# bingjeff/trex-gym

Measured on NVIDIA B200. Metric: env-steps/sec at 65,536 envs/GPU, higher is better.
Workload: dtype f32

## Files before the change

### trex_gym_b200/csrc/trex_core.h

```cpp
#pragma once
#include "trex_topology.h"
#include <stddef.h>

#ifndef TREX_KMAX
#define TREX_KMAX 16
#endif
#ifndef TREX_PGS_UNROLL
#define TREX_PGS_UNROLL TREX_ROLLED
#endif
#define TREX_NCAND_MAX 64
#define TREX_MAX_ROUNDS 12
#ifdef TREX_PHASES
#define TREX_STATE_STRIDE 176
#else
#define TREX_STATE_STRIDE 160
#endif
#define W_COL 0
#define W_RHSM 992
#define W_JDI 1024
#define W_DSELF 1056
#define W_RHSL 1088
#define W_SIGMA 1120
#define TREX_KC 8
#define W_NC 1152
#define W_CS 1160
#define W_BT (W_CS + 16 * TREX_KC)
#define W_A4 (W_BT + 96 * TREX_KC)
#define TREX_WORK_STRIDE 2848
static_assert(W_A4 + 12 * TREX_KC * TREX_KC <= TREX_WORK_STRIDE && (W_BT % 4) == 0 && (W_A4 % 4) == 0 && (TREX_WORK_STRIDE % 32) == 0,
              "work record layout");
#define TREX_KW TREX_KMAX
#define H_NC 0
#define H_CS 8
#define H_BT (H_CS + 16 * TREX_KW)
#define H_A4 (H_BT + 96 * TREX_KW)
#define TREX_HEAVY_STRIDE (((H_A4 + 9 * TREX_KW * TREX_KW) + 31) / 32 * 32)
static_assert((H_BT % 4) == 0 && (H_A4 % 4) == 0 && TREX_KC <= TREX_KW, "heavy record layout");
#define TREX_NCLASS 6
#define TREX_CLASS_HEAVY (TREX_NCLASS - 1)
TREX_TOPO_FN int defer_class(int n_contacts) {
  return n_contacts <= 2 ? n_contacts : (n_contacts <= 4 ? 3 : (n_contacts <= TREX_KC ? 4 : TREX_CLASS_HEAVY));
}
#ifdef TREX_PHASES
#define TREX_AUX_STRIDE 16
#define TREX_TICK(i) { const long long _t = cycle_count(); stats.phase[i] += (float)(_t - _t0); _t0 = _t; }
#else
#define TREX_AUX_STRIDE 8
#define TREX_TICK(i)
#endif

namespace trex {

using trex_topo::NB;
using trex_topo::NJ;
using trex_topo::MAX_DEPTH;

enum {
  F_E0 = 0,
  F_R0 = 9,
  F_MASS = 12,
  F_MC = 13,
  F_I = 16,
  F_DROT = 22,
  F_LOWER = 28,
  F_UPPER = 29,
  F_JDAMP = 30,
  F_STARTQ = 31,
  F_COUNT = 32
};
enum {
  IF_PARENT_LANE = 0,
  IF_DEPTH = 1,
  IF_ANC_MASK = 2,
  IF_CHILDREN = 3,
  IF_OBS_SLOT = 4,
  IF_DAMP_LANE = 5,
  IF_DAMP_CONTRIB = 6,
  IF_LIMIT_ORDER = 7,
  IF_LEVEL = 8,
  IF_COUNT = 8 + MAX_DEPTH
};

struct Uniform {
  float dt, g, kp, kd, max_impulse, k_lin, k_ang, maxvel, erp, contact_erp, split_thresh, slop;
  float resid_thresh, warm, mu, breaking, floor_z, limit_max_impulse, reset_z, target_h;
  float w_dist, w_energy, w_drift;
  float head_p[3];
  float r0[NB][3];
  int iters, n_sub, max_episode_steps, head_lane, n_cand, n_rounds, contacts_on, reset_mode;
  int defer_contacts;
  unsigned seed;
  long long env_offset;
  float reset_z_min, reset_z_max;
  unsigned char order[2 * NJ];
  unsigned char depth[NB];
  unsigned char max_children[MAX_DEPTH + 1];
  unsigned char head_chain[MAX_DEPTH];
  int head_depth;
};

struct alignas(16) WarpShared {
  float col[31][32];
  float tmp[1][32];
  float lam_cache[TREX_NCAND_MAX];
  float cpos[TREX_KMAX][4];
  int ccand[TREX_KMAX];
  int clane[TREX_KMAX];
  union {
    struct {
      float E[9][32];
      float U[6][32];
      float invD[32];
      float Rw[9][32];
      float xw[3][32];
      float pack[32][16];
    } k;
    struct {
      float dV[3 * TREX_KMAX][32];
      float Jc[3 * TREX_KMAX][12];
      unsigned char slot[TREX_KMAX][32];
      unsigned char inv[TREX_KW][16];
    } c;
    struct {
      float keep[28][32];
      float pA[6][32];
      float cc[5][32];
      float uu[32];
      float Ip[21][32];
      float pp[6][32];
      float base[32];
    } x;
  };
};
static_assert(sizeof(((WarpShared*)0)->x) <= sizeof(((WarpShared*)0)->c), "exchange area must fit the union");
static_assert(sizeof(((WarpShared*)0)->x.keep) == 28 * 128, "exchange area must start behind k.E .. k.xw");
#define TREX_PART_ROW 44
static_assert(sizeof(((WarpShared*)0)->k) <= TREX_PART_ROW * 128, "partials must not overlap the kinematics arrays");
static_assert(sizeof(((WarpShared*)0)->c) >= (TREX_PART_ROW + 6) * 128, "contact-row storage too small for the damping scratch");

TREX_FN constexpr int SI(int i, int j) {
  return (i <= j) ? (i * 6 - (i * (i - 1)) / 2 + (j - i)) : (j * 6 - (j * (j - 1)) / 2 + (i - j));
}
TREX_FN constexpr int body_lane(int b) { return b == 0 ? 25 : b - 1; }

struct EnvRegs {
  vf q, qd, tgt, tau;
  float pos[3], quat[4], om[3], vl[3];
};

TREX_FN uint32_t sig_mix_u(uint32_t h, uint32_t w) { return (h ^ w) * 16777619u; }
#define TREX_CONE_EDGE 0.9999f

struct StepStats {
  uint32_t sig;
  int iters;
  int contacts;
  int overflow;
#ifdef TREX_PHASES
  float phase[8];
#endif
};

#define MDL(f) ldg_ro(mdl, lane + (f) * 32)
#define MDLI(f) ldi(mdli, lane + (f) * 32)

TREX_FN vf clampv(vf x, float lo, float hi) { return sel(x < lo, lo, sel(x > hi, hi, x)); }
TREX_FN float clampf(float x, float lo, float hi) { return x < lo ? lo : (x > hi ? hi : x); }

TREX_FN void quat_to_Rb(const float q[4], float Rb[9]) {
  const float x = q[0], y = q[1], z = q[2], w = q[3];
  const float s = 2.0f / (x * x + y * y + z * z + w * w);
  Rb[0] = 1.0f - s * (y * y + z * z); Rb[3] = s * (x * y - w * z);        Rb[6] = s * (x * z + w * y);
  Rb[1] = s * (x * y + w * z);        Rb[4] = 1.0f - s * (x * x + z * z); Rb[7] = s * (y * z - w * x);
  Rb[2] = s * (x * z - w * y);        Rb[5] = s * (y * z + w * x);        Rb[8] = 1.0f - s * (x * x + y * y);
}

TREX_FN void local_rotation(const float* mdl, vi lane, vf q, vf E[9]) {
  const vf c = vcos(q), s = vsin(q);
  vf e0[9];
  TREX_UNROLL for (int k = 0; k < 9; k++) e0[k] = MDL(F_E0 + k);
  E[0] = c * e0[0] + s * e0[1]; E[1] = c * e0[3] + s * e0[4]; E[2] = c * e0[6] + s * e0[7];
  E[3] = c * e0[1] - s * e0[0]; E[4] = c * e0[4] - s * e0[3]; E[5] = c * e0[7] - s * e0[6];
  E[6] = e0[2]; E[7] = e0[5]; E[8] = e0[8];
}

template <bool WITH_VEL>
TREX_FN void forward_pass(const float* mdl, const int* mdli, vi lane, const EnvRegs& R, const float Rb[9],
                          const vf E[9], vf Rw[9], vf xw[3], vf v[6]) {
  const vi plane = MDLI(IF_PARENT_LANE);
  const vi depth = MDLI(IF_DEPTH);
  vf r0[3];
  TREX_UNROLL for (int k = 0; k < 3; k++) r0[k] = MDL(F_R0 + k);
  TREX_UNROLL for (int k = 0; k < 9; k++) Rw[k] = vbroadcast(Rb[k]);
  TREX_UNROLL for (int k = 0; k < 3; k++) xw[k] = vbroadcast(R.pos[k]);
  if (WITH_VEL) {
    TREX_UNROLL for (int i = 0; i < 3; i++) {
      v[i] = vbroadcast(Rb[3 * i] * R.om[0] + Rb[3 * i + 1] * R.om[1] + Rb[3 * i + 2] * R.om[2]);
      v[3 + i] = vbroadcast(Rb[3 * i] * R.vl[0] + Rb[3 * i + 1] * R.vl[1] + Rb[3 * i + 2] * R.vl[2]);
    }
  }
  TREX_ROLLED for (int d = 1; d <= MAX_DEPTH; d++) {
    const vb at = depth == d;
    vf pR[9], px[3];
    TREX_UNROLL for (int k = 0; k < 9; k++) pR[k] = shflv(Rw[k], plane);
    TREX_UNROLL for (int k = 0; k < 3; k++) px[k] = shflv(xw[k], plane);
    TREX_UNROLL for (int i = 0; i < 3; i++)
      TREX_UNROLL for (int j = 0; j < 3; j++) {
        const vf t = E[3 * i] * pR[j] + E[3 * i + 1] * pR[3 + j] + E[3 * i + 2] * pR[6 + j];
        Rw[3 * i + j] = sel(at, t, Rw[3 * i + j]);
      }
    TREX_UNROLL for (int j = 0; j < 3; j++) {
      const vf t = px[j] + pR[j] * r0[0] + pR[3 + j] * r0[1] + pR[6 + j] * r0[2];
      xw[j] = sel(at, t, xw[j]);
    }
    if (WITH_VEL) {
      vf pv[6];
      TREX_UNROLL for (int k = 0; k < 6; k++) pv[k] = shflv(v[k], plane);
      const vf lx = pv[3] + (pv[1] * r0[2] - pv[2] * r0[1]);
      const vf ly = pv[4] + (pv[2] * r0[0] - pv[0] * r0[2]);
      const vf lz = pv[5] + (pv[0] * r0[1] - pv[1] * r0[0]);
      TREX_UNROLL for (int i = 0; i < 3; i++) {
        vf wa = E[3 * i] * pv[0] + E[3 * i + 1] * pv[1] + E[3 * i + 2] * pv[2];
        const vf la = E[3 * i] * lx + E[3 * i + 1] * ly + E[3 * i + 2] * lz;
        if (i == 2) wa = wa + R.qd;
        v[i] = sel(at, wa, v[i]);
        v[3 + i] = sel(at, la, v[3 + i]);
      }
    }
  }
}

struct Chol6 {
  float L[6][6];
  float rd[6];
};
TREX_FN void spd6_factor(const float a[21], Chol6& c) {
  TREX_UNROLL for (int j = 0; j < 6; j++) {
    float s = a[SI(j, j)];
    TREX_UNROLL for (int k = 0; k < j; k++) s -= c.L[j][k] * c.L[j][k];
    const float id = 1.0f / sqrtf(s);
    c.rd[j] = id;
    TREX_UNROLL for (int i = j + 1; i < 6; i++) {
      float t = a[SI(i, j)];
      TREX_UNROLL for (int k = 0; k < j; k++) t -= c.L[i][k] * c.L[j][k];
      c.L[i][j] = t * id;
    }
  }
}
template <class T>
TREX_FN void spd6_solve_neg(const Chol6& c, const T b[6], T x[6]) {
  T y[6];
  TREX_UNROLL for (int i = 0; i < 6; i++) {
    T t = b[i];
    TREX_UNROLL for (int k = 0; k < i; k++) t = t - y[k] * c.L[i][k];
    y[i] = t * c.rd[i];
  }
  TREX_UNROLL for (int i = 5; i >= 0; i--) {
    T t = y[i];
    TREX_UNROLL for (int k = i + 1; k < 6; k++) t = t - x[k] * c.L[k][i];
    x[i] = t * c.rd[i];
  }
  TREX_UNROLL for (int i = 0; i < 6; i++) x[i] = -x[i];
}

TREX_FN void to_parent(const vf E[9], const vf r[3], const vf Ia[21], const vf pa[6], vf Ip[21], vf pp[6]) {
  vf Ar[3][3], Br[3][3], Mr[3][3];
  {
    const vf a00 = Ia[SI(0, 0)], a01 = Ia[SI(0, 1)], a11 = Ia[SI(1, 1)];
    vf T0[3], T1[3];
    TREX_UNROLL for (int j = 0; j < 3; j++) {
      T0[j] = a00 * E[j] + a01 * E[3 + j];
      T1[j] = a01 * E[j] + a11 * E[3 + j];
    }
    TREX_UNROLL for (int i = 0; i < 3; i++)
      TREX_UNROLL for (int j = i; j < 3; j++) Ar[i][j] = E[i] * T0[j] + E[3 + i] * T1[j];
  }
  {
    vf T0[3], T1[3];
    TREX_UNROLL for (int j = 0; j < 3; j++) {
      T0[j] = Ia[SI(0, 3)] * E[j] + Ia[SI(0, 4)] * E[3 + j] + Ia[SI(0, 5)] * E[6 + j];
      T1[j] = Ia[SI(1, 3)] * E[j] + Ia[SI(1, 4)] * E[3 + j] + Ia[SI(1, 5)] * E[6 + j];
    }
    TREX_UNROLL for (int i = 0; i < 3; i++)
      TREX_UNROLL for (int j = 0; j < 3; j++) Br[i][j] = E[i] * T0[j] + E[3 + i] * T1[j];
  }
  {
    vf T[3][3];
    TREX_UNROLL for (int i = 0; i < 3; i++)
      TREX_UNROLL for (int j = 0; j < 3; j++)
        T[i][j] = Ia[SI(3 + i, 3)] * E[j] + Ia[SI(3 + i, 4)] * E[3 + j] + Ia[SI(3 + i, 5)] * E[6 + j];
    TREX_UNROLL for (int i = 0; i < 3; i++)
      TREX_UNROLL for (int j = i; j < 3; j++) {
        Mr[i][j] = E[i] * T[0][j] + E[3 + i] * T[1][j] + E[6 + i] * T[2][j];
        Mr[j][i] = Mr[i][j];
      }
  }
  vf K[3][3], C[3][3], Dm[3][3], Bp[3][3];
  TREX_UNROLL for (int j = 0; j < 3; j++) {
    K[0][j] = r[1] * Mr[2][j] - r[2] * Mr[1][j];
    K[1][j] = r[2] * Mr[0][j] - r[0] * Mr[2][j];
    K[2][j] = r[0] * Mr[1][j] - r[1] * Mr[0][j];
  }
  TREX_UNROLL for (int i = 0; i < 3; i++)
    TREX_UNROLL for (int j = 0; j < 3; j++) Bp[i][j] = Br[i][j] + K[i][j];
  TREX_UNROLL for (int j = 0; j < 3; j++) {
    C[0][j] = r[1] * Br[j][2] - r[2] * Br[j][1];
    C[1][j] = r[2] * Br[j][0] - r[0] * Br[j][2];
    C[2][j] = r[0] * Br[j][1] - r[1] * Br[j][0];
    Dm[0][j] = r[1] * Bp[j][2] - r[2] * Bp[j][1];
    Dm[1][j] = r[2] * Bp[j][0] - r[0] * Bp[j][2];
    Dm[2][j] = r[0] * Bp[j][1] - r[1] * Bp[j][0];
  }
  TREX_UNROLL for (int i = 0; i < 3; i++)
    TREX_UNROLL for (int j = i; j < 3; j++) {
      Ip[SI(i, j)] = Ar[i][j] + C[i][j] + Dm[j][i];
      Ip[SI(3 + i, 3 + j)] = Mr[i][j];
    }
  TREX_UNROLL for (int i = 0; i < 3; i++)
    TREX_UNROLL for (int j = 0; j < 3; j++) Ip[SI(i, 3 + j)] = Bp[i][j];
  vf fn[3], ff[3];
  TREX_UNROLL for (int i = 0; i < 3; i++) {
    fn[i] = E[i] * pa[0] + E[3 + i] * pa[1] + E[6 + i] * pa[2];
    ff[i] = E[i] * pa[3] + E[3 + i] * pa[4] + E[6 + i] * pa[5];
  }
  pp[0] = fn[0] + (r[1] * ff[2] - r[2] * ff[1]);
  pp[1] = fn[1] + (r[2] * ff[0] - r[0] * ff[2]);
  pp[2] = fn[2] + (r[0] * ff[1] - r[1] * ff[0]);
  pp[3] = ff[0]; pp[4] = ff[1]; pp[5] = ff[2];
}

TREX_FN void finish_substep(const Uniform& P, vi lane, EnvRegs& R, vf dv, vf lam_m) {
  const vb is_joint = lane < NJ;
  const float dt = P.dt;
  R.qd = sel(is_joint, clampv(R.qd + dv, -P.maxvel, P.maxvel), 0.0f);
  TREX_UNROLL for (int k = 0; k < 3; k++) {
    R.om[k] = clampf(R.om[k] + lane_value(dv, 25 + k), -P.maxvel, P.maxvel);
    R.vl[k] = clampf(R.vl[k] + lane_value(dv, 28 + k), -P.maxvel, P.maxvel);
  }
  R.tau = sel(is_joint, vdiv(lam_m, dt), 0.0f);
  TREX_UNROLL for (int k = 0; k < 3; k++) R.pos[k] += dt * R.vl[k];
  {
    float fAngle = sqrtf(R.om[0] * R.om[0] + R.om[1] * R.om[1] + R.om[2] * R.om[2]);
    if (fAngle * dt > 0.78539816339744831f) fAngle = 0.78539816339744831f / dt;
    float sc;
    if (fAngle < 0.001f) sc = 0.5f * dt - (dt * dt * dt) * 0.020833333333f * fAngle * fAngle;
    else sc = sinf(0.5f * fAngle * dt) / fAngle;
    const float ax = R.om[0] * sc, ay = R.om[1] * sc, az = R.om[2] * sc, aw = cosf(fAngle * dt * 0.5f);
    const float x = R.quat[0], y = R.quat[1], z = R.quat[2], w = R.quat[3];
    const float nx = aw * x + ax * w + ay * z - az * y;
    const float ny = aw * y - ax * z + ay * w + az * x;
    const float nz = aw * z + ax * y - ay * x + az * w;
    const float nw = aw * w - ax * x - ay * y - az * z;
    const float inv = 1.0f / sqrtf(nx * nx + ny * ny + nz * nz + nw * nw);
    R.quat[0] = nx * inv; R.quat[1] = ny * inv; R.quat[2] = nz * inv; R.quat[3] = nw * inv;
  }
  R.q = sel(is_joint, R.q + dt * R.qd, 0.0f);
}

TREX_FN void inward_packed(const Uniform& P, const float* mdl, const int* mdli, WarpShared* slabs, int valid_mask) {
  const vi lane = lane_id();
  const vi e = lane >> 3, i = lane & 7;
  const vb env_ok = ((vi(valid_mask) >> e) & 1) != 0;
  float* sb = reinterpret_cast<float*>(slabs);
  const vi eo = e * (int)(sizeof(WarpShared) / sizeof(float));
  constexpr int O_E = offsetof(WarpShared, k.E) / 4, O_U = offsetof(WarpShared, k.U) / 4, O_ID = offsetof(WarpShared, k.invD) / 4;
  constexpr int O_PA = offsetof(WarpShared, x.pA) / 4, O_CC = offsetof(WarpShared, x.cc) / 4, O_UU = offsetof(WarpShared, x.uu) / 4;
  constexpr int O_IP = offsetof(WarpShared, x.Ip) / 4, O_PP = offsetof(WarpShared, x.pp) / 4, O_BASE = offsetof(WarpShared, x.base) / 4;
  vi blv[MAX_DEPTH + 1];
  blv[0] = seli(i == 0, vi(25), vi(-1));
  TREX_UNROLL for (int d = 1; d <= MAX_DEPTH; d++) blv[d] = ldi(mdli, i + (IF_LEVEL + d - 1) * 32);
  vf n_mass, n_mc[3], n_I3[6], n_r0[3];
  vi n_children;
#define TREX_LOAD_LEVEL_CONSTANTS(BL)                                                       \
  {                                                                                         \
    const vi b_ = (BL);                                                                     \
    n_mass = ldg_ro(mdl, b_ + F_MASS * 32);                                                 \
    TREX_UNROLL for (int k = 0; k < 3; k++) n_mc[k] = ldg_ro(mdl, b_ + (F_MC + k) * 32);    \
    TREX_UNROLL for (int k = 0; k < 6; k++) n_I3[k] = ldg_ro(mdl, b_ + (F_I + k) * 32);     \
    TREX_UNROLL for (int k = 0; k < 3; k++) n_r0[k] = ldg_ro(mdl, b_ + (F_R0 + k) * 32);    \
    n_children = ldi(mdli, b_ + IF_CHILDREN * 32);                                          \
  }
  TREX_LOAD_LEVEL_CONSTANTS(seli(env_ok && (blv[MAX_DEPTH] >= 0), blv[MAX_DEPTH], 0))
  TREX_ROLLED for (int d = MAX_DEPTH; d >= 0; d--) {
    vi bl0 = blv[0], bln = blv[0];
    TREX_UNROLL for (int dd = 1; dd <= MAX_DEPTH; dd++) {
      bl0 = seli(vi(d) == dd, blv[dd], bl0);
      bln = seli(vi(d) == dd + 1, blv[dd], bln);
    }
    const vb has = env_ok && (bl0 >= 0);
    const vi bl = seli(has, bl0, 0);
    vf mc[3], I3[6], r0[3], pA[6];
    const vf mass = n_mass;
    const vi children = n_children;
    TREX_UNROLL for (int k = 0; k < 3; k++) { mc[k] = n_mc[k]; r0[k] = n_r0[k]; }
    TREX_UNROLL for (int k = 0; k < 6; k++) I3[k] = n_I3[k];
    if (d > 0) TREX_LOAD_LEVEL_CONSTANTS(seli(env_ok && (bln >= 0), bln, 0))
    TREX_UNROLL for (int k = 0; k < 6; k++) pA[k] = ld(sb, eo + bl + (O_PA + k * 32));
    vf IA[21];
    TREX_UNROLL for (int k = 0; k < 21; k++) IA[k] = 0.0f;
    IA[SI(0, 0)] = I3[0]; IA[SI(0, 1)] = I3[1]; IA[SI(0, 2)] = I3[2];
    IA[SI(1, 1)] = I3[3]; IA[SI(1, 2)] = I3[4]; IA[SI(2, 2)] = I3[5];
    IA[SI(0, 4)] = -mc[2]; IA[SI(0, 5)] = mc[1];
    IA[SI(1, 3)] = mc[2];  IA[SI(1, 5)] = -mc[0];
    IA[SI(2, 3)] = -mc[1]; IA[SI(2, 4)] = mc[0];
    IA[SI(3, 3)] = mass; IA[SI(4, 4)] = mass; IA[SI(5, 5)] = mass;
    if (d < MAX_DEPTH) {
      const int nslots = P.max_children[d];
      TREX_ROLLED for (int sidx = 0; sidx < nslots; sidx++) {
        const vi cl = (children >> (6 * sidx)) & 63;
        const vb ok = has && (cl != 63);
        const vi cls = seli(ok, cl, bl);
        TREX_UNROLL for (int k = 0; k < 21; k++) IA[k] = IA[k] + sel(ok, ld(sb, eo + cls + (O_IP + k * 32)), 0.0f);
        TREX_UNROLL for (int k = 0; k < 6; k++) pA[k] = pA[k] + sel(ok, ld(sb, eo + cls + (O_PP + k * 32)), 0.0f);
      }
    }
    if (d == 0) {
      TREX_UNROLL for (int k = 0; k < 21; k++) st_if(sb, eo + (O_BASE + k), IA[k], has);
      TREX_UNROLL for (int k = 0; k < 6; k++) st_if(sb, eo + (O_BASE + 21 + k), pA[k], has);
      break;
    }
    vf E[9];
    TREX_UNROLL for (int k = 0; k < 9; k++) E[k] = ld(sb, eo + bl + (O_E + k * 32));
    const vf c0 = ld(sb, eo + bl + O_CC), c1 = ld(sb, eo + bl + (O_CC + 32)), c3 = ld(sb, eo + bl + (O_CC + 64)),
             c4 = ld(sb, eo + bl + (O_CC + 96)), tau_j = ld(sb, eo + bl + (O_CC + 128));
    vf Ut[6];
    Ut[0] = IA[SI(0, 2)]; Ut[1] = IA[SI(1, 2)]; Ut[2] = IA[SI(2, 2)];
    Ut[3] = IA[SI(2, 3)]; Ut[4] = IA[SI(2, 4)]; Ut[5] = IA[SI(2, 5)];
    const vf Dt = Ut[2];
    const vb okD = Dt >= 1.1920929e-7f;
    const vf iD = sel(okD, vdiv(1.0f, sel(okD, Dt, 1.0f)), 0.0f);
    const vf ut = tau_j - pA[2];
    TREX_UNROLL for (int k = 0; k < 6; k++) st_if(sb, eo + bl + (O_U + k * 32), Ut[k], has);
    st_if(sb, eo + bl + O_ID, iD, has);
    st_if(sb, eo + bl + O_UU, ut, has);
    vf Ia[21];
    TREX_UNROLL for (int a = 0; a < 6; a++)
      TREX_UNROLL for (int b = a; b < 6; b++) Ia[SI(a, b)] = IA[SI(a, b)] - (Ut[a] * iD) * Ut[b];
    vf pa[6];
    const vf s = ut * iD;
    TREX_UNROLL for (int a = 0; a < 6; a++)
      pa[a] = a == 2 ? pA[a] + Ut[a] * s : pA[a] + (Ia[SI(a, 0)] * c0 + Ia[SI(a, 1)] * c1 + Ia[SI(a, 3)] * c3 + Ia[SI(a, 4)] * c4) + Ut[a] * s;
    vf Ip[21], pp[6];
    to_parent(E, r0, Ia, pa, Ip, pp);
    TREX_UNROLL for (int k = 0; k < 21; k++) st_if(sb, eo + bl + (O_IP + k * 32), Ip[k], has);
    TREX_UNROLL for (int k = 0; k < 6; k++) st_if(sb, eo + bl + (O_PP + k * 32), pp[k], has);
    warp_sync();
  }
#undef TREX_LOAD_LEVEL_CONSTANTS
  warp_sync();
}

template <bool PACKED = false>
TREX_FN int substep(const Uniform& P, const float* mdl, const int* mdli, const float* tasks, const float* cand_p,
                     const int* cand_lane, WarpShared& S, EnvRegs& R, float kp, float kd, float max_imp,
                     StepStats& stats, float* work, WarpShared* cta_slabs = nullptr, int warp_in_cta = 0, int valid_mask = 0,
                     float* workh = nullptr) {
  const vi lane = lane_id();
  const vb is_joint = lane < NJ;
  const vb is_base = lane == 25;
  const vi plane = MDLI(IF_PARENT_LANE);
  const vi depth = MDLI(IF_DEPTH);
  const vi anc = MDLI(IF_ANC_MASK);
  const float dt = P.dt;

#ifdef TREX_PHASES
  long long _t0 = cycle_count();
#endif
  float Rb[9];
  quat_to_Rb(R.quat, Rb);

  vf E[9];
  local_rotation(mdl, lane, R.q, E);
  TREX_UNROLL for (int k = 0; k < 9; k++) E[k] = sel(is_base, vbroadcast(Rb[k]), E[k]);
  vf Rw[9], xw[3], v[6];
  forward_pass<true>(mdl, mdli, lane, R, Rb, E, Rw, xw, v);
  TREX_UNROLL for (int k = 0; k < 9; k++) { st(S.k.E[k], lane, E[k]); st(S.k.Rw[k], lane, Rw[k]); }
  TREX_UNROLL for (int k = 0; k < 3; k++) st(S.k.xw[k], lane, xw[k]);

  TREX_TICK(0)
  const vf mass = MDL(F_MASS);
  vf mc[3], I3[6];
  TREX_UNROLL for (int k = 0; k < 3; k++) mc[k] = MDL(F_MC + k);
  TREX_UNROLL for (int k = 0; k < 6; k++) I3[k] = MDL(F_I + k);
  vf pA[6];
  {
    const vf wx = v[0], wy = v[1], wz = v[2], lx = v[3], ly = v[4], lz = v[5];
    const vf nx = I3[0] * wx + I3[1] * wy + I3[2] * wz + (mc[1] * lz - mc[2] * ly);
    const vf ny = I3[1] * wx + I3[3] * wy + I3[4] * wz + (mc[2] * lx - mc[0] * lz);
    const vf nz = I3[2] * wx + I3[4] * wy + I3[5] * wz + (mc[0] * ly - mc[1] * lx);
    const vf fx = mass * lx - (mc[1] * wz - mc[2] * wy);
    const vf fy = mass * ly - (mc[2] * wx - mc[0] * wz);
    const vf fz = mass * lz - (mc[0] * wy - mc[1] * wx);
    pA[0] = (wy * nz - wz * ny) + (ly * fz - lz * fy);
    pA[1] = (wz * nx - wx * nz) + (lz * fx - lx * fz);
    pA[2] = (wx * ny - wy * nx) + (lx * fy - ly * fx);
    pA[3] = wy * fz - wz * fy;
    pA[4] = wz * fx - wx * fz;
    pA[5] = wx * fy - wy * fx;
    const vf gx = -P.g * Rw[2], gy = -P.g * Rw[5], gz = -P.g * Rw[8];
    pA[0] -= mc[1] * gz - mc[2] * gy;
    pA[1] -= mc[2] * gx - mc[0] * gz;
    pA[2] -= mc[0] * gy - mc[1] * gx;
    pA[3] -= mass * gx; pA[4] -= mass * gy; pA[5] -= mass * gz;
    vf dr[6];
    TREX_UNROLL for (int k = 0; k < 6; k++) dr[k] = MDL(F_DROT + k);
    const vf wn = vsqrt(wx * wx + wy * wy + wz * wz);
    const vf ka = P.k_ang + P.k_ang * wn;
    pA[0] += (dr[0] * wx + dr[1] * wy + dr[2] * wz) * ka;
    pA[1] += (dr[1] * wx + dr[3] * wy + dr[4] * wz) * ka;
    pA[2] += (dr[2] * wx + dr[4] * wy + dr[5] * wz) * ka;
  }
  {
    const vi dl = MDLI(IF_DAMP_LANE);
    vf bv[6];
    TREX_UNROLL for (int k = 0; k < 6; k++) bv[k] = shflv(v[k], dl);
    vf acc[6];
    TREX_UNROLL for (int k = 0; k < 6; k++) acc[k] = 0.0f;
    _Pragma("unroll 5") for (int rd = 0; rd < P.n_rounds; rd++) {
      const float* t = tasks + rd * 4 * 32;
      const vf rx = ldg_ro(t, lane), ry = ldg_ro(t, lane + 32), rz = ldg_ro(t, lane + 64), m = ldg_ro(t, lane + 96);
      const vf cx = bv[3] + (bv[1] * rz - bv[2] * ry);
      const vf cy = bv[4] + (bv[2] * rx - bv[0] * rz);
      const vf cz = bv[5] + (bv[0] * ry - bv[1] * rx);
      const vf sc = m * (P.k_lin + P.k_lin * vsqrt(cx * cx + cy * cy + cz * cz));
      const vf fx = cx * sc, fy = cy * sc, fz = cz * sc;
      acc[0] += ry * fz - rz * fy;
      acc[1] += rz * fx - rx * fz;
      acc[2] += rx * fy - ry * fx;
      acc[3] += fx; acc[4] += fy; acc[5] += fz;
    }
    warp_sync();
    TREX_UNROLL for (int k = 0; k < 6; k++) st(reinterpret_cast<float*>(&S.c) + (TREX_PART_ROW + k) * 32, lane, acc[k]);
    warp_sync();
    const vi contrib = MDLI(IF_DAMP_CONTRIB);
    TREX_UNROLL for (int s = 0; s < 4; s++) {
      const vi cl = (contrib >> (6 * s)) & 63;
      const vb ok = cl != 63;
      const vi cls = seli(ok, cl, lane);
      TREX_UNROLL for (int k = 0; k < 6; k++) pA[k] += sel(ok, ld(reinterpret_cast<float*>(&S.c) + (TREX_PART_ROW + k) * 32, cls), 0.0f);
    }
    warp_sync();
  }

  const vf c0 = R.qd * v[1], c1 = -(R.qd * v[0]), c3 = R.qd * v[4], c4 = -(R.qd * v[3]);
  const vf tau_j = -(MDL(F_JDAMP) * R.qd);

  TREX_TICK(1)
  vf IA[21];
  TREX_UNROLL for (int k = 0; k < 21; k++) IA[k] = 0.0f;
  IA[SI(0, 0)] = I3[0]; IA[SI(0, 1)] = I3[1]; IA[SI(0, 2)] = I3[2];
  IA[SI(1, 1)] = I3[3]; IA[SI(1, 2)] = I3[4]; IA[SI(2, 2)] = I3[5];
  IA[SI(0, 4)] = -mc[2]; IA[SI(0, 5)] = mc[1];
  IA[SI(1, 3)] = mc[2];  IA[SI(1, 5)] = -mc[0];
  IA[SI(2, 3)] = -mc[1]; IA[SI(2, 4)] = mc[0];
  IA[SI(3, 3)] = mass; IA[SI(4, 4)] = mass; IA[SI(5, 5)] = mass;
  vf r0[3];
  TREX_UNROLL for (int k = 0; k < 3; k++) r0[k] = MDL(F_R0 + k);
  const vi children = MDLI(IF_CHILDREN);
  vf U[6], invD = 0.0f, uu = 0.0f;
  TREX_UNROLL for (int k = 0; k < 6; k++) U[k] = 0.0f;
  if (PACKED) {
    TREX_UNROLL for (int k = 0; k < 6; k++) st(S.x.pA[k], lane, pA[k]);
    st(S.x.cc[0], lane, c0); st(S.x.cc[1], lane, c1); st(S.x.cc[2], lane, c3); st(S.x.cc[3], lane, c4); st(S.x.cc[4], lane, tau_j);
    cta_sync();
    if (warp_in_cta == 0) inward_packed(P, mdl, mdli, cta_slabs, valid_mask);
    cta_sync();
    TREX_UNROLL for (int k = 0; k < 6; k++) U[k] = sel(is_joint, ld(S.k.U[k], lane), 0.0f);
    invD = sel(is_joint, ld(S.k.invD, lane), 0.0f);
    uu = sel(is_joint, ld(S.x.uu, lane), 0.0f);
  }
  TREX_ROLLED for (int d = PACKED ? 0 : MAX_DEPTH; d >= 1; d--) {
    const vb at = depth == d;
    vf Ut[6];
    Ut[0] = IA[SI(0, 2)]; Ut[1] = IA[SI(1, 2)]; Ut[2] = IA[SI(2, 2)];
    Ut[3] = IA[SI(2, 3)]; Ut[4] = IA[SI(2, 4)]; Ut[5] = IA[SI(2, 5)];
    const vf Dt = Ut[2];
    const vb okD = Dt >= 1.1920929e-7f;
    const vf iD = sel(okD, vdiv(1.0f, sel(okD, Dt, 1.0f)), 0.0f);
    const vf ut = tau_j - pA[2];
    TREX_UNROLL for (int k = 0; k < 6; k++) U[k] = sel(at, Ut[k], U[k]);
    invD = sel(at, iD, invD);
    uu = sel(at, ut, uu);
    vf Ia[21];
    TREX_UNROLL for (int i = 0; i < 6; i++)
      TREX_UNROLL for (int j = i; j < 6; j++) Ia[SI(i, j)] = IA[SI(i, j)] - (Ut[i] * iD) * Ut[j];
    vf pa[6];
    const vf s = ut * iD;
    TREX_UNROLL for (int i = 0; i < 6; i++)
      pa[i] = i == 2 ? pA[i] + Ut[i] * s : pA[i] + (Ia[SI(i, 0)] * c0 + Ia[SI(i, 1)] * c1 + Ia[SI(i, 3)] * c3 + Ia[SI(i, 4)] * c4) + Ut[i] * s;
    vf Ip[21], pp[6];
    to_parent(E, r0, Ia, pa, Ip, pp);
    const vb parent_now = depth == (d - 1);
    const int nslots = P.max_children[d - 1];
    TREX_ROLLED for (int sidx = 0; sidx < nslots; sidx++) {
      const vi cl = (children >> (6 * sidx)) & 63;
      const vb ok = parent_now && (cl != 63);
      const vi cls = seli(ok, cl, lane);
      const vf okf = sel(ok, 1.0f, 0.0f);
      TREX_UNROLL for (int k = 0; k < 21; k++) IA[k] = vfma(okf, shflv(Ip[k], cls), IA[k]);
      TREX_UNROLL for (int k = 0; k < 6; k++) pA[k] = vfma(okf, shflv(pp[k], cls), pA[k]);
    }
  }
  float ia0[21], pA0[6], a0[6];
  if (PACKED) {
    TREX_UNROLL for (int k = 0; k < 21; k++) ia0[k] = ldu(S.x.base, k);
    TREX_UNROLL for (int k = 0; k < 6; k++) pA0[k] = ldu(S.x.base, 21 + k);
    warp_sync();
  } else {
    TREX_UNROLL for (int k = 0; k < 21; k++) ia0[k] = lane_value(IA[k], 25);
    TREX_UNROLL for (int k = 0; k < 6; k++) pA0[k] = lane_value(pA[k], 25);
    TREX_UNROLL for (int k = 0; k < 6; k++) st(S.k.U[k], lane, U[k]);
    st(S.k.invD, lane, invD);
  }
  {
    vf pk[16];
    TREX_UNROLL for (int k = 0; k < 9; k++) pk[k] = E[k];
    TREX_UNROLL for (int k = 0; k < 6; k++) pk[9 + k] = U[k];
    pk[15] = invD;
    st16(&S.k.pack[0][0], lane * 16, pk);
  }

  TREX_TICK(2)
  Chol6 chol0;
  spd6_factor(ia0, chol0);
  spd6_solve_neg<float>(chol0, pA0, a0);

  vf a[6];
  TREX_UNROLL for (int k = 0; k < 6; k++) a[k] = vbroadcast(a0[k]);
  vf qdd = 0.0f;
  TREX_ROLLED for (int d = 1; d <= MAX_DEPTH; d++) {
    const vb at = depth == d;
    vf ap[6];
    TREX_UNROLL for (int k = 0; k < 6; k++) ap[k] = shflv(a[k], plane);
    const vf lx = ap[3] + (ap[1] * r0[2] - ap[2] * r0[1]);
    const vf ly = ap[4] + (ap[2] * r0[0] - ap[0] * r0[2]);
    const vf lz = ap[5] + (ap[0] * r0[1] - ap[1] * r0[0]);
    vf an[6];
    TREX_UNROLL for (int i = 0; i < 3; i++) {
      an[i] = E[3 * i] * ap[0] + E[3 * i + 1] * ap[1] + E[3 * i + 2] * ap[2];
      an[3 + i] = E[3 * i] * lx + E[3 * i + 1] * ly + E[3 * i + 2] * lz;
    }
    an[0] += c0; an[1] += c1; an[3] += c3; an[4] += c4;
    const vf dd = (uu - (U[0] * an[0] + U[1] * an[1] + U[2] * an[2] + U[3] * an[3] + U[4] * an[4] + U[5] * an[5])) * invD;
    an[2] += dd;
    qdd = sel(at, dd, qdd);
    TREX_UNROLL for (int k = 0; k < 6; k++) a[k] = sel(at, an[k], a[k]);
  }

  R.qd = sel(is_joint, clampv(R.qd + dt * qdd, -P.maxvel, P.maxvel), 0.0f);
  {
    const float wb[3] = {Rb[0] * R.om[0] + Rb[1] * R.om[1] + Rb[2] * R.om[2], Rb[3] * R.om[0] + Rb[4] * R.om[1] + Rb[5] * R.om[2],
                         Rb[6] * R.om[0] + Rb[7] * R.om[1] + Rb[8] * R.om[2]};
    const float vb_[3] = {Rb[0] * R.vl[0] + Rb[1] * R.vl[1] + Rb[2] * R.vl[2], Rb[3] * R.vl[0] + Rb[4] * R.vl[1] + Rb[5] * R.vl[2],
                          Rb[6] * R.vl[0] + Rb[7] * R.vl[1] + Rb[8] * R.vl[2]};
    const float al[3] = {a0[3] + (wb[1] * vb_[2] - wb[2] * vb_[1]), a0[4] + (wb[2] * vb_[0] - wb[0] * vb_[2]),
                         a0[5] + (wb[0] * vb_[1] - wb[1] * vb_[0])};
    TREX_UNROLL for (int j = 0; j < 3; j++) {
      const float wd = Rb[j] * a0[0] + Rb[3 + j] * a0[1] + Rb[6 + j] * a0[2];
      const float vd = Rb[j] * al[0] + Rb[3 + j] * al[1] + Rb[6 + j] * al[2];
      R.om[j] = clampf(R.om[j] + dt * wd, -P.maxvel, P.maxvel);
      R.vl[j] = clampf(R.vl[j] + dt * vd, -P.maxvel, P.maxvel);
    }
  }
  warp_sync();

  TREX_TICK(3)
  {
    vf z[6];
    TREX_UNROLL for (int k = 0; k < 6; k++) z[k] = sel(is_joint, U[k] * invD, 0.0f);
    vf Ydep[MAX_DEPTH + 1];
    TREX_UNROLL for (int dd = 0; dd <= MAX_DEPTH; dd++) Ydep[dd] = sel(is_joint && (depth == dd), 1.0f, 0.0f);
    vi cur = lane;
    TREX_ROLLED for (int s = 0; s < MAX_DEPTH; s++) {
      const vb active = is_joint && ((depth - s) >= 1);
      const vi cs = seli(active, cur, lane);
      vf Ec[9], rc[3];
      TREX_UNROLL for (int k = 0; k < 9; k++) Ec[k] = ld(S.k.E[k], cs);
      TREX_UNROLL for (int k = 0; k < 3; k++) rc[k] = ldg_ro(mdl, cs + (F_R0 + k) * 32);
      vf fn[3], ff[3];
      TREX_UNROLL for (int i = 0; i < 3; i++) {
        fn[i] = Ec[i] * z[0] + Ec[3 + i] * z[1] + Ec[6 + i] * z[2];
        ff[i] = Ec[i] * z[3] + Ec[3 + i] * z[4] + Ec[6 + i] * z[5];
      }
      vf zn[6];
      zn[0] = fn[0] + (rc[1] * ff[2] - rc[2] * ff[1]);
      zn[1] = fn[1] + (rc[2] * ff[0] - rc[0] * ff[2]);
      zn[2] = fn[2] + (rc[0] * ff[1] - rc[1] * ff[0]);
      zn[3] = ff[0]; zn[4] = ff[1]; zn[5] = ff[2];
      const vi par = ldi(mdli, cs + IF_PARENT_LANE * 32);
      const vb par_joint = active && (par != 25);
      const vi ps = seli(par_joint, par, lane);
      const vf Yp = -zn[2];
      const vf sc = Yp * ld(S.k.invD, ps);
      TREX_UNROLL for (int k = 0; k < 6; k++) {
        const vf up = ld(S.k.U[k], ps);
        z[k] = sel(active, sel(par_joint, zn[k] + up * sc, zn[k]), z[k]);
      }
      const vi pd = depth - s - 1;
      TREX_UNROLL for (int dd = 1; dd <= MAX_DEPTH; dd++) Ydep[dd] = sel(par_joint && (pd == dd), Yp, Ydep[dd]);
      cur = seli(active, par, cur);
    }
    {
      const vi kk = lane - 25;
      TREX_UNROLL for (int k = 0; k < 3; k++) {
        const vf rk = sel(kk == 0 || kk == 3, vbroadcast(Rb[3 * k]), sel(kk == 1 || kk == 4, vbroadcast(Rb[3 * k + 1]), vbroadcast(Rb[3 * k + 2])));
        const vb isw = (lane >= 25) && (lane < 28);
        const vb isv = (lane >= 28) && (lane < 31);
        z[k] = sel(isw, -rk, sel(is_joint, z[k], 0.0f));
        z[3 + k] = sel(isv, -rk, sel(is_joint, z[3 + k], 0.0f));
      }
    }
    vf astk[MAX_DEPTH + 1][6];
    spd6_solve_neg<vf>(chol0, z, astk[0]);
    TREX_UNROLL for (int dd = 1; dd <= MAX_DEPTH; dd++)
      TREX_UNROLL for (int k = 0; k < 6; k++) astk[dd][k] = 0.0f;
    TREX_ROLLED for (int b = 1; b < NB; b++) {
      const int bl = b - 1;
      const int dep = P.depth[b];
      float pk[16];
      ldu16(&S.k.pack[0][0], bl * 16, pk);
      const float* Eb = pk;
      const float* Ub = pk + 9;
      const float iDb = pk[15];
      const float rx = P.r0[b][0], ry = P.r0[b][1], rz = P.r0[b][2];
      const vb onpath = ((anc >> bl) & 1) != 0;
      vf ddq = 0.0f;
#define TREX_COL_BODY(D)                                                                              \
      {                                                                                               \
        const vf* ap = astk[(D) - 1];                                                                 \
        vf* an = astk[(D)];                                                                           \
        const vf lx = ap[3] + (ap[1] * rz - ap[2] * ry);                                              \
        const vf ly = ap[4] + (ap[2] * rx - ap[0] * rz);                                              \
        const vf lz = ap[5] + (ap[0] * ry - ap[1] * rx);                                              \
        vf t[6];                                                                                      \
        TREX_UNROLL for (int i = 0; i < 3; i++) {                                                     \
          t[i] = Eb[3 * i] * ap[0] + Eb[3 * i + 1] * ap[1] + Eb[3 * i + 2] * ap[2];                   \
          t[3 + i] = Eb[3 * i] * lx + Eb[3 * i + 1] * ly + Eb[3 * i + 2] * lz;                        \
        }                                                                                             \
        const vf Yb = sel(onpath, Ydep[(D)], 0.0f);                                                   \
        ddq = (Yb - (Ub[0] * t[0] + Ub[1] * t[1] + Ub[2] * t[2] + Ub[3] * t[3] + Ub[4] * t[4] + Ub[5] * t[5])) * iDb; \
        t[2] += ddq;                                                                                  \
        TREX_UNROLL for (int k = 0; k < 6; k++) an[k] = t[k];                                         \
      }
      switch (dep) {
        case 1: TREX_COL_BODY(1) break;
        case 2: TREX_COL_BODY(2) break;
        case 3: TREX_COL_BODY(3) break;
        case 4: TREX_COL_BODY(4) break;
        default: TREX_COL_BODY(5) break;
      }
#undef TREX_COL_BODY
      st(S.col[6 + bl], lane, ddq);
    }
    TREX_UNROLL for (int j = 0; j < 3; j++) {
      st(S.col[j], lane, Rb[j] * astk[0][0] + Rb[3 + j] * astk[0][1] + Rb[6 + j] * astk[0][2]);
      st(S.col[3 + j], lane, Rb[j] * astk[0][3] + Rb[3 + j] * astk[0][4] + Rb[6 + j] * astk[0][5]);
    }
  }
  warp_sync();

  TREX_TICK(4)
  vi c_bl[2];
  vf c_px[2], c_py[2], c_pz[2], c_pr[2];
  TREX_UNROLL for (int half = 0; half < 2; half++) {
    const vi ci = lane + 32 * half;
    const vi cis = seli(ci < P.n_cand, ci, 0);
    c_bl[half] = ldi(cand_lane, cis);
    c_px[half] = ldg_ro(cand_p, cis); c_py[half] = ldg_ro(cand_p, cis + TREX_NCAND_MAX);
    c_pz[half] = ldg_ro(cand_p, cis + 2 * TREX_NCAND_MAX); c_pr[half] = ldg_ro(cand_p, cis + 3 * TREX_NCAND_MAX);
  }
  vf uown = R.qd;
  vf dself = 0.0f;
  TREX_UNROLL for (int k = 0; k < 3; k++) {
    uown = sel(lane == 25 + k, vbroadcast(R.om[k]), uown);
    uown = sel(lane == 28 + k, vbroadcast(R.vl[k]), uown);
  }
  uown = sel(lane == 31, 0.0f, uown);
  {
    const vi gown = seli(is_joint, lane + 6, seli(lane < 31, lane - 25, 0));
    dself = sel(lane < 31, ld(&S.col[0][0], gown * 32 + lane), 0.0f);
  }
  const vb okJ = is_joint && (dself > 1.1920929e-7f);
  const vf jdi = sel(okJ, vdiv(1.0f, sel(okJ, dself, 1.0f)), 0.0f);
  const vf vt = kp * (R.tgt - R.q) / dt + R.qd + kd * (0.0f - R.qd);
  const vf rhs_m = (vt - R.qd) * jdi;
  vf lam_m = 0.0f;
  vf lamr[NJ];
  TREX_UNROLL for (int j = 0; j < NJ; j++) lamr[j] = 0.0f;
  const vf lower = MDL(F_LOWER), upper = MDL(F_UPPER);
  const vf pen_lo = R.q - lower, pen_hi = upper - R.q;
  const vb act_lo = is_joint && !(pen_lo > 0.0f);
  const vb act_hi = is_joint && !(pen_hi > 0.0f);
  const vf rhs_lo = sel(pen_lo > P.split_thresh, (-pen_lo * P.erp / dt + (-R.qd)) * jdi, (-R.qd) * jdi);
  const vf rhs_hi = sel(pen_hi > P.split_thresh, (-pen_hi * P.erp / dt + (R.qd)) * jdi, (R.qd) * jdi);
  vf lam_lo = 0.0f, lam_hi = 0.0f;
  const uint32_t mask_lo = vballot(act_lo), mask_hi = vballot(act_hi);
  uint32_t lim_perm;
  {
    const vi pj = ldi(mdli, lane + IF_LIMIT_ORDER * 32);
    lim_perm = vballot((lane < NJ) && ((((vi((int)(mask_lo | mask_hi))) >> pj) & 1) != 0));
  }

  int n_act = 0;
  vf c_lam[3], c_rhs[3], c_jdi[3], c_dd[3];
  TREX_UNROLL for (int k = 0; k < 3; k++) { c_lam[k] = 0.0f; c_rhs[k] = 0.0f; c_jdi[k] = 0.0f; c_dd[k] = 0.0f; }
  vf dv = 0.0f;
  if (P.contacts_on) {
    vf wpos[2][3];
    vi cbl[2];
    vb cact[2];
    uint32_t am[2];
    TREX_UNROLL for (int half = 0; half < 2; half++) {
      const vi ci = lane + 32 * half;
      const vb valid = ci < P.n_cand;
      const vi cis = seli(valid, ci, 0);
      const vi bl = c_bl[half];
      const vf px = c_px[half], py = c_py[half], pz = c_pz[half];
      wpos[half][0] = ld(S.k.xw[0], bl) + ld(S.k.Rw[0], bl) * px + ld(S.k.Rw[3], bl) * py + ld(S.k.Rw[6], bl) * pz;
      wpos[half][1] = ld(S.k.xw[1], bl) + ld(S.k.Rw[1], bl) * px + ld(S.k.Rw[4], bl) * py + ld(S.k.Rw[7], bl) * pz;
      wpos[half][2] = (ld(S.k.xw[2], bl) + ld(S.k.Rw[2], bl) * px + ld(S.k.Rw[5], bl) * py + ld(S.k.Rw[8], bl) * pz) - c_pr[half];
      cbl[half] = bl;
      cact[half] = valid && ((wpos[half][2] - P.floor_z) < P.breaking);
      am[half] = vballot(cact[half]);
    }
    const int total = popc_u(am[0]) + popc_u(am[1]);
    if (total > TREX_KMAX) {
      stats.overflow += total - TREX_KMAX;
      TREX_UNROLL for (int half = 0; half < 2; half++) {
        vi better = 0;
        TREX_UNROLL for (int h2 = 0; h2 < 2; h2++) {
          TREX_ROLLED for (int l2 = 0; l2 < 32; l2++) {
            if (!((am[h2] >> l2) & 1u)) continue;
            const float z2 = lane_value(wpos[h2][2], l2);
            const vi idx2 = vi(l2 + 32 * h2), idx = lane + 32 * half;
            better = better + seli((z2 < wpos[half][2]) || ((z2 == wpos[half][2]) && (idx2 < idx)), vi(1), vi(0));
          }
        }
        cact[half] = cact[half] && (better < TREX_KMAX);
      }
      am[0] = vballot(cact[0]);
      am[1] = vballot(cact[1]);
    }
    TREX_UNROLL for (int half = 0; half < 2; half++) {
      const vi ci = lane + 32 * half;
      const vb valid = ci < P.n_cand;
      const vi cis = seli(valid, ci, 0);
      const vi rank = rank_below(am[half]) + n_act;
      const vb keep = cact[half];
      const vi slot = seli(keep, rank, 0);
      st_if(&S.cpos[0][0], slot * 4 + 0, wpos[half][0], keep);
      st_if(&S.cpos[0][0], slot * 4 + 1, wpos[half][1], keep);
      st_if(&S.cpos[0][0], slot * 4 + 2, wpos[half][2], keep);
      sti_if(S.ccand, slot, ci, keep);
      sti_if(S.clane, slot, cbl[half], keep);
      st_if(S.lam_cache, cis, 0.0f, valid && !keep);
      n_act += popc_u(am[half]);
    }
    warp_sync();
    stats.sig = sig_mix_u(sig_mix_u(stats.sig, am[0]), am[1]) & 0xffffffu;
  } else {
    stats.sig = sig_mix_u(sig_mix_u(stats.sig, 0u), 0u) & 0xffffffu;
  }
  const bool defer_c = work != nullptr && P.defer_contacts != 0 && n_act > 0 && n_act <= ((P.defer_contacts > 1 && workh != nullptr) ? TREX_KW : TREX_KC);
  if (work != nullptr && (n_act == 0 || defer_c)) {
    _Pragma("unroll 8") for (int gq = 0; gq < trex_topo::NDOF; gq++) st(work, lane + (W_COL + gq * 32), ld(S.col[gq], lane));
    st(work, lane + W_RHSM, rhs_m);
    st(work, lane + W_JDI, jdi);
    st(work, lane + W_DSELF, sel(is_joint, dself, 0.0f));
    st(work, lane + W_RHSL, sel(act_lo, rhs_lo, sel(act_hi, rhs_hi, 0.0f)));
    st(work, lane + W_SIGMA, sel(act_lo, 1.0f, sel(act_hi, -1.0f, 0.0f)));
    stats.contacts = n_act;
    if (n_act == 0) {
      warp_sync();
      TREX_TICK(5)
      return 1;
    }
  }
  if (P.contacts_on) {
    const vf ax = Rw[6], ay = Rw[7], az = Rw[8];
    const vi mydepth = seli(is_joint, depth, 0);
    TREX_ROLLED for (int c = 0; c < n_act; c++) {
      const float Px = ldu(&S.cpos[0][0], 4 * c), Py = ldu(&S.cpos[0][0], 4 * c + 1), Pz = ldu(&S.cpos[0][0], 4 * c + 2);
      const int cl = ldui(S.clane, c);
      const int cc = ldui(S.ccand, c);
      const int ancb = cl == 25 ? 0 : lane_value_i(anc, cl);
      const vb moves = is_joint && (((vi(ancb) >> lane) & 1) != 0);
      const vf ex = Px - xw[0], ey = Py - xw[1], ez = Pz - xw[2];
      const vf jx = sel(moves, ay * ez - az * ey, 0.0f);
      const vf jy = sel(moves, az * ex - ax * ez, 0.0f);
      const vf jz = sel(moves, ax * ey - ay * ex, 0.0f);
      const float bx = Px - R.pos[0], by = Py - R.pos[1], bz = Pz - R.pos[2];
      vf Jn = jz, J1 = -jy, J2 = jx;
      Jn = sel(lane == 25, by, sel(lane == 26, -bx, sel(lane == 30, 1.0f, Jn)));
      J1 = sel(lane == 25, bz, sel(lane == 27, -bx, sel(lane == 29, -1.0f, J1)));
      J2 = sel(lane == 26, bz, sel(lane == 27, -by, sel(lane == 28, 1.0f, J2)));
      const vf Jr[3] = {Jn, J1, J2};
      const vb isb = (lane >= 25) && (lane < 31);
      const vi myslot = seli(isb, lane - 25, seli(moves, mydepth + 5, 11));
      warp_sync();
      if (defer_c) {
        TREX_UNROLL for (int k = 0; k < 3; k++) st_if(S.c.Jc[3 * c + k], seli(lane < 12, lane, 0), 0.0f, lane < 12);
        stb(S.c.inv[c], lane & 15, vi(31));
        warp_sync();
      }
// ... 1365 lines not shown
```

Baseline: 8.774 million.

## Split articulated-body inward pass into inertia and bias-force sweeps via shared memory

The non-packed inward recursion is split into two depth sweeps. The first propagates articulated inertias and caches the per-link Ia·c coupling term. The second propagates only the 6-component bias forces using the cached U, invD and coupling. Child-to-parent transfer now goes through shared-memory stores and loads instead of warp shuffles with FMA masking. This shortens each sweep's live register set, at the cost of an extra depth loop, extra warp syncs and shared-memory traffic. It relies on S.x having Ip and pp fields.

```diff
diff --git a/trex_gym_b200/csrc/trex_core.h b/trex_gym_b200/csrc/trex_core.h
--- a/trex_gym_b200/csrc/trex_core.h
+++ b/trex_gym_b200/csrc/trex_core.h
@@ -263,7 +263,7 @@
   TREX_UNROLL for (int i = 0; i < 6; i++) x[i] = -x[i];
 }
 
-TREX_FN void to_parent(const vf E[9], const vf r[3], const vf Ia[21], const vf pa[6], vf Ip[21], vf pp[6]) {
+TREX_FN void inertia_to_parent(const vf E[9], const vf r[3], const vf Ia[21], vf Ip[21]) {
   vf Ar[3][3], Br[3][3], Mr[3][3];
   {
     const vf a00 = Ia[SI(0, 0)], a01 = Ia[SI(0, 1)], a11 = Ia[SI(1, 1)];
@@ -318,6 +318,8 @@
     }
   TREX_UNROLL for (int i = 0; i < 3; i++)
     TREX_UNROLL for (int j = 0; j < 3; j++) Ip[SI(i, 3 + j)] = Bp[i][j];
+}
+TREX_FN void force_to_parent(const vf E[9], const vf r[3], const vf pa[6], vf pp[6]) {
   vf fn[3], ff[3];
   TREX_UNROLL for (int i = 0; i < 3; i++) {
     fn[i] = E[i] * pa[0] + E[3 + i] * pa[1] + E[6 + i] * pa[2];
@@ -441,7 +443,8 @@
     TREX_UNROLL for (int a = 0; a < 6; a++)
       pa[a] = a == 2 ? pA[a] + Ut[a] * s : pA[a] + (Ia[SI(a, 0)] * c0 + Ia[SI(a, 1)] * c1 + Ia[SI(a, 3)] * c3 + Ia[SI(a, 4)] * c4) + Ut[a] * s;
     vf Ip[21], pp[6];
-    to_parent(E, r0, Ia, pa, Ip, pp);
+    inertia_to_parent(E, r0, Ia, Ip);
+    force_to_parent(E, r0, pa, pp);
     TREX_UNROLL for (int k = 0; k < 21; k++) st_if(sb, eo + bl + (O_IP + k * 32), Ip[k], has);
     TREX_UNROLL for (int k = 0; k < 6; k++) st_if(sb, eo + bl + (O_PP + k * 32), pp[k], has);
     warp_sync();
@@ -568,38 +571,58 @@
     TREX_UNROLL for (int k = 0; k < 6; k++) U[k] = sel(is_joint, ld(S.k.U[k], lane), 0.0f);
     invD = sel(is_joint, ld(S.k.invD, lane), 0.0f);
     uu = sel(is_joint, ld(S.x.uu, lane), 0.0f);
-  }
-  TREX_ROLLED for (int d = PACKED ? 0 : MAX_DEPTH; d >= 1; d--) {
-    const vb at = depth == d;
-    vf Ut[6];
-    Ut[0] = IA[SI(0, 2)]; Ut[1] = IA[SI(1, 2)]; Ut[2] = IA[SI(2, 2)];
-    Ut[3] = IA[SI(2, 3)]; Ut[4] = IA[SI(2, 4)]; Ut[5] = IA[SI(2, 5)];
-    const vf Dt = Ut[2];
-    const vb okD = Dt >= 1.1920929e-7f;
-    const vf iD = sel(okD, vdiv(1.0f, sel(okD, Dt, 1.0f)), 0.0f);
-    const vf ut = tau_j - pA[2];
-    TREX_UNROLL for (int k = 0; k < 6; k++) U[k] = sel(at, Ut[k], U[k]);
-    invD = sel(at, iD, invD);
-    uu = sel(at, ut, uu);
-    vf Ia[21];
-    TREX_UNROLL for (int i = 0; i < 6; i++)
-      TREX_UNROLL for (int j = i; j < 6; j++) Ia[SI(i, j)] = IA[SI(i, j)] - (Ut[i] * iD) * Ut[j];
-    vf pa[6];
-    const vf s = ut * iD;
-    TREX_UNROLL for (int i = 0; i < 6; i++)
-      pa[i] = i == 2 ? pA[i] + Ut[i] * s : pA[i] + (Ia[SI(i, 0)] * c0 + Ia[SI(i, 1)] * c1 + Ia[SI(i, 3)] * c3 + Ia[SI(i, 4)] * c4) + Ut[i] * s;
-    vf Ip[21], pp[6];
-    to_parent(E, r0, Ia, pa, Ip, pp);
-    const vb parent_now = depth == (d - 1);
-    const int nslots = P.max_children[d - 1];
-    TREX_ROLLED for (int sidx = 0; sidx < nslots; sidx++) {
-      const vi cl = (children >> (6 * sidx)) & 63;
-      const vb ok = parent_now && (cl != 63);
-      const vi cls = seli(ok, cl, lane);
-      const vf okf = sel(ok, 1.0f, 0.0f);
-      TREX_UNROLL for (int k = 0; k < 21; k++) IA[k] = vfma(okf, shflv(Ip[k], cls), IA[k]);
-      TREX_UNROLL for (int k = 0; k < 6; k++) pA[k] = vfma(okf, shflv(pp[k], cls), pA[k]);
-    }
+  } else {
+    vf Iac[6];
+    TREX_UNROLL for (int k = 0; k < 6; k++) Iac[k] = 0.0f;
+    TREX_ROLLED for (int d = MAX_DEPTH; d >= 1; d--) {
+      const vb at = depth == d;
+      vf Ut[6];
+      Ut[0] = IA[SI(0, 2)]; Ut[1] = IA[SI(1, 2)]; Ut[2] = IA[SI(2, 2)];
+      Ut[3] = IA[SI(2, 3)]; Ut[4] = IA[SI(2, 4)]; Ut[5] = IA[SI(2, 5)];
+      const vf Dt = Ut[2];
+      const vb okD = Dt >= 1.1920929e-7f;
+      const vf iD = sel(okD, vdiv(1.0f, sel(okD, Dt, 1.0f)), 0.0f);
+      TREX_UNROLL for (int k = 0; k < 6; k++) U[k] = sel(at, Ut[k], U[k]);
+      invD = sel(at, iD, invD);
+      vf Ia[21];
+      TREX_UNROLL for (int i = 0; i < 6; i++)
+        TREX_UNROLL for (int j = i; j < 6; j++) Ia[SI(i, j)] = IA[SI(i, j)] - (Ut[i] * iD) * Ut[j];
+      TREX_UNROLL for (int i = 0; i < 6; i++)
+        if (i != 2) Iac[i] = sel(at, Ia[SI(i, 0)] * c0 + Ia[SI(i, 1)] * c1 + Ia[SI(i, 3)] * c3 + Ia[SI(i, 4)] * c4, Iac[i]);
+      vf Ip[21];
+      inertia_to_parent(E, r0, Ia, Ip);
+      TREX_UNROLL for (int k = 0; k < 21; k++) st_if(S.x.Ip[k], lane, Ip[k], at);
+      warp_sync();
+      const vb parent_now = depth == (d - 1);
+      const int nslots = P.max_children[d - 1];
+      TREX_ROLLED for (int sidx = 0; sidx < nslots; sidx++) {
+        const vi cl = (children >> (6 * sidx)) & 63;
+        const vb ok = parent_now && (cl != 63);
+        const vi cls = seli(ok, cl, lane);
+        TREX_UNROLL for (int k = 0; k < 21; k++) IA[k] = sel(ok, IA[k] + ld(S.x.Ip[k], cls), IA[k]);
+      }
+    }
+    TREX_ROLLED for (int d = MAX_DEPTH; d >= 1; d--) {
+      const vb at = depth == d;
+      const vf ut = tau_j - pA[2];
+      uu = sel(at, ut, uu);
+      const vf s = ut * invD;
+      vf pa[6];
+      TREX_UNROLL for (int i = 0; i < 6; i++) pa[i] = i == 2 ? pA[i] + U[i] * s : (pA[i] + Iac[i]) + U[i] * s;
+      vf pp[6];
+      force_to_parent(E, r0, pa, pp);
+      TREX_UNROLL for (int k = 0; k < 6; k++) st_if(S.x.pp[k], lane, pp[k], at);
+      warp_sync();
+      const vb parent_now = depth == (d - 1);
+      const int nslots = P.max_children[d - 1];
+      TREX_ROLLED for (int sidx = 0; sidx < nslots; sidx++) {
+        const vi cl = (children >> (6 * sidx)) & 63;
+        const vb ok = parent_now && (cl != 63);
+        const vi cls = seli(ok, cl, lane);
+        TREX_UNROLL for (int k = 0; k < 6; k++) pA[k] = sel(ok, pA[k] + ld(S.x.pp[k], cls), pA[k]);
+      }
+    }
+    warp_sync();
   }
   float ia0[21], pA0[6], a0[6];
   if (PACKED) {
```

Measured after the change: 8.913 million (median of 6 runs). 1.02x the previous value.
